# sMedX/FaceNet

Measured on AMD Instinct MI355X. Metric: images/sec (160x160 triplet train), higher is better.
Workload: dtype bf16

## Files before the change

### facenet_amd/csrc/common.h

```cpp
#pragma once
#include <hip/hip_runtime.h>
#include <stdint.h>
#include <atomic>
#include <cstdlib>

namespace fn {

enum { FN_OK = 0, FN_EINVAL = -1, FN_ELAUNCH = -2, FN_EUNSUPPORTED = -3 };
void set_error(const char* fmt, ...);
int check_launch(const char* what);

#define FN_REQUIRE(cond, ...)                  \
    do {                                       \
        if (!(cond)) {                         \
            fn::set_error(__VA_ARGS__);        \
            return fn::FN_EINVAL;              \
        }                                      \
    } while (0)

typedef __attribute__((ext_vector_type(8))) __bf16 bf16x8;
typedef __attribute__((ext_vector_type(4))) __bf16 bf16x4;
typedef __attribute__((ext_vector_type(8))) _Float16 f16x8;
typedef __attribute__((ext_vector_type(4))) _Float16 f16x4;
typedef __attribute__((ext_vector_type(4))) float f32x4;
// ... 19 lines not shown
    static __device__ __forceinline__ f32x4 mfma(vec8 a, vec8 b, f32x4 c) {
        return __builtin_amdgcn_mfma_f32_16x16x32_bf16(a, b, c, 0, 0, 0);
    }
};
template <> struct LP<_Float16> {
    typedef f16x8 vec8;
    typedef f16x4 vec4;
    static __device__ __forceinline__ float to_f32(unsigned short b) { return (float)__builtin_bit_cast(_Float16, b); }
    static __device__ __forceinline__ unsigned short from_f32(float f) {
        _Float16 h = (_Float16)f;
        return __builtin_bit_cast(unsigned short, h);
    }
    static __device__ __forceinline__ f32x4 mfma(vec8 a, vec8 b, f32x4 c) {
        return __builtin_amdgcn_mfma_f32_16x16x32_f16(a, b, c, 0, 0, 0);
    }
};

template <typename T> __device__ __forceinline__ void unpack8(const u32x4& v, float (&f)[8]) {
#pragma unroll
    for (int i = 0; i < 4; ++i) {
        f[2 * i] = LP<T>::to_f32((unsigned short)(v[i] & 0xffffu));
        f[2 * i + 1] = LP<T>::to_f32((unsigned short)(v[i] >> 16));
    }
}
template <typename T> __device__ __forceinline__ u32x4 pack8(const float (&f)[8]) {
    u32x4 v;
#pragma unroll
    for (int i = 0; i < 4; ++i)
        v[i] = (unsigned)LP<T>::from_f32(f[2 * i]) | ((unsigned)LP<T>::from_f32(f[2 * i + 1]) << 16);
    return v;
}

__device__ __forceinline__ void fast_divmod(int m, int d, float inv, int& q, int& r) {
    q = (int)((float)m * inv);
    r = m - q * d;
    const int lo = r < 0 ? 1 : 0, hi = r >= d ? 1 : 0;
    q += hi - lo;
    r += (lo - hi) * d;
}

__device__ __forceinline__ float wave_sum(float v) {
#pragma unroll
    for (int o = 32; o > 0; o >>= 1) v += __shfl_xor(v, o);
    return v;
}
__device__ __forceinline__ float wave_max(float v) {
#pragma unroll
    for (int o = 32; o > 0; o >>= 1) v = fmaxf(v, __shfl_xor(v, o));
    return v;
}

typedef int64_t acc_t;
enum { ACC_STAT = 20, ACC_GRAD = 40 };
template <int FRAC> __device__ __forceinline__ void acc_add(acc_t* p, float v) {
    atomicAdd(reinterpret_cast<unsigned long long*>(p), (unsigned long long)__double2ll_rn((double)v * (double)(1ll << FRAC)));
}
template <int FRAC> __device__ __forceinline__ float acc_get(acc_t a) { return (float)((double)a * (1.0 / (double)(1ll << FRAC))); }

__device__ __forceinline__ void bn_affine_from_sums(float s1, float s2, int count, float eps, float beta, float& scale, float& shift,
                                                    float& mean, float& var) {
#pragma clang fp contract(off)
    const float inv = 1.f / (float)count;
    mean = s1 * inv;
    const float ex2 = s2 * inv, m2 = mean * mean;
    var = fmaxf(ex2 - m2, 0.f);
    scale = rsqrtf(var + eps);
    const float ms = mean * scale;
    shift = beta - ms;
}

__device__ __forceinline__ float bn_moving_update(float moving, float batch, float momentum) {
#pragma clang fp contract(off)
    const float a = moving * momentum, w = 1.f - momentum;
    const float b = batch * w;
    return a + b;
}

__device__ __forceinline__ void bn_batch_affine(const acc_t* __restrict__ stats, int c, int sq_off, int reps, int rep_stride, int count,
                                                float eps, float beta, float& scale, float& shift, float& mean, float& var) {
    acc_t s = 0, q = 0;
    for (int rp = 0; rp < reps; ++rp) {
        s += stats[(long)rp * rep_stride + c];
        q += stats[(long)rp * rep_stride + sq_off + c];
    }
    bn_affine_from_sums(acc_get<ACC_STAT>(s), acc_get<ACC_STAT>(q), count, eps, beta, scale, shift, mean, var);
}

enum { STORE_WT = 17 };
__device__ __forceinline__ __amdgpu_buffer_rsrc_t wt_rsrc(const void* base) {
    return __builtin_amdgcn_make_buffer_rsrc(const_cast<void*>(base), 0, 0x7fffffff, 0x00020000);
}
__device__ __forceinline__ void store_wt(const __amdgpu_buffer_rsrc_t rs, long byte_offset, u32x4 v) {
    __builtin_amdgcn_raw_buffer_store_b128(v, rs, (int)byte_offset, 0, STORE_WT);
}

__device__ __forceinline__ int xcd_remap(int bid, int nwg) {
    const int q = nwg >> 3, r = nwg & 7, x = bid & 7;
    const int base = (x < r) ? x * (q + 1) : r * (q + 1) + (x - r) * q;
    return base + (bid >> 3);
}

static inline int cdiv(long a, long b) { return (int)((a + b - 1) / b); }

static inline int env_int(const char* name, int dflt) {
    const char* v = getenv(name);
    return v ? atoi(v) : dflt;
}

struct LdsOptIn {
    std::atomic<bool> done[32];
};
static inline int allow_big_lds(const void* kernel, LdsOptIn& state, const char* what) {
    int dev = 0;
    if (hipGetDevice(&dev) != hipSuccess || dev < 0 || dev >= 32) {
        set_error("%s: no current HIP device (or more than 32 devices)", what);
        return FN_ELAUNCH;
    }
    if (state.done[dev].load(std::memory_order_relaxed)) return FN_OK;
    const hipError_t e = hipFuncSetAttribute(kernel, hipFuncAttributeMaxDynamicSharedMemorySize, 160 * 1024);
    if (e != hipSuccess) {
        set_error("%s: hipFuncSetAttribute(MaxDynamicSharedMemorySize, 160 KiB) failed on device %d: %s", what, dev, hipGetErrorString(e));
        return FN_ELAUNCH;
    }
    state.done[dev].store(true, std::memory_order_relaxed);
    return FN_OK;
}

static __global__ void fill_words_kernel(unsigned* __restrict__ p, unsigned v0, unsigned v1, int n) {
    for (int i = blockIdx.x * blockDim.x + threadIdx.x; i < n; i += gridDim.x * blockDim.x) p[i] = (i & 1) ? v1 : v0;
}
static inline void fill_words(void* p, unsigned v0, unsigned v1, int n, hipStream_t st) {
    hipLaunchKernelGGL(fill_words_kernel, dim3(n > 4096 ? 16 : 1), dim3(256), 0, st, (unsigned*)p, v0, v1, n);
}

}
```

### facenet_amd/csrc/elementwise.hip

```cpp
#include "common.h"
#include "../../include/facenet_hip.h"

namespace fn {

__device__ __forceinline__ unsigned f2ord(float f) {
    unsigned u = __float_as_uint(f);
    return (u & 0x80000000u) ? ~u : (u | 0x80000000u);
}
__device__ __forceinline__ float ord2f(unsigned u) {
    return __uint_as_float((u & 0x80000000u) ? (u & 0x7fffffffu) : ~u);
}

template <typename SRC>
__global__ __launch_bounds__(256) void img_stats_kernel(const SRC* __restrict__ img, unsigned* __restrict__ work, int count) {
    const int n = blockIdx.y;
    const SRC* p = img + (long)n * count;
    float mx = -3e38f, mn = 3e38f, s = 0.f, q = 0.f;
    constexpr int PER = 16 / sizeof(SRC);
    const int head = min(count, (int)(((16 - ((uintptr_t)p & 15)) & 15) / sizeof(SRC)));
    const int nvec = (count - head) / PER;
    const SRC* pv = p + head;
    for (int i = blockIdx.x * 256 + threadIdx.x; i < nvec; i += gridDim.x * 256) {
        const u32x4 v = *reinterpret_cast<const u32x4*>(pv + (long)i * PER);
#pragma unroll
        for (int w = 0; w < 4; ++w) {
            if constexpr (sizeof(SRC) == 1) {
#pragma unroll
                for (int b = 0; b < 4; ++b) {
                    const float x = (float)((v[w] >> (8 * b)) & 0xffu);
                    mx = fmaxf(mx, x); mn = fminf(mn, x); s += x; q += x * x;
                }
            } else {
                const float x = __uint_as_float(v[w]);
                mx = fmaxf(mx, x); mn = fminf(mn, x); s += x; q += x * x;
            }
        }
    }
    if (blockIdx.x == 0) {
        for (int i = threadIdx.x; i < head; i += 256) {
            const float x = (float)p[i];
            mx = fmaxf(mx, x); mn = fminf(mn, x); s += x; q += x * x;
        }
        for (int i = head + nvec * PER + threadIdx.x; i < count; i += 256) {
            const float x = (float)p[i];
            mx = fmaxf(mx, x); mn = fminf(mn, x); s += x; q += x * x;
        }
    }
    mx = wave_max(mx); mn = -wave_max(-mn); s = wave_sum(s); q = wave_sum(q);
    if ((threadIdx.x & 63) == 0) {
        atomicMax(&work[8 * n + 0], f2ord(mx));
        atomicMax(&work[8 * n + 1], f2ord(-mn));
        acc_add<ACC_STAT>(reinterpret_cast<acc_t*>(&work[8 * n + 2]), s);
        acc_add<ACC_STAT>(reinterpret_cast<acc_t*>(&work[8 * n + 4]), q);
    }
}

template <typename T, typename SRC>
__global__ __launch_bounds__(256) void img_apply_kernel(const SRC* __restrict__ img, unsigned short* __restrict__ out,
                                                        const unsigned* __restrict__ work, int HW, int mode) {
    const int n = blockIdx.y;
    float mul, sub, den;
    if (mode == 0) {
        const float mx = ord2f(work[8 * n + 0]), mn = -ord2f(work[8 * n + 1]);
        mul = 2.f; sub = mn + mx; den = fmaxf(mx - mn, 1e-3f);
    } else {
        const float cnt = (float)HW * 3.f;
        const float mean = acc_get<ACC_STAT>(*reinterpret_cast<const acc_t*>(&work[8 * n + 2])) / cnt;
        const float var = fmaxf(acc_get<ACC_STAT>(*reinterpret_cast<const acc_t*>(&work[8 * n + 4])) / cnt - mean * mean, 0.f);
        mul = 1.f; sub = mean; den = fmaxf(sqrtf(var), rsqrtf(cnt));
    }
    const SRC* p = img + (long)n * HW * 3;
    unsigned short* o = out + (long)n * HW * 8;
    for (int px = blockIdx.x * 256 + threadIdx.x; px < HW; px += gridDim.x * 256) {
        float v[8] = {0, 0, 0, 0, 0, 0, 0, 0};
#pragma unroll
        for (int c = 0; c < 3; ++c) v[c] = (mul * (float)p[px * 3 + c] - sub) / den;
        *reinterpret_cast<u32x4*>(o + (long)px * 8) = pack8<T>(v);
    }
}

template <typename SRC>
__global__ __launch_bounds__(256) void resize_bilinear_kernel(const SRC* __restrict__ img, float* __restrict__ out, int N, int H, int W,
                                                              int OH, int OW) {
    const float sy = (float)H / (float)OH, sx = (float)W / (float)OW;
    const long total = (long)N * OH * OW;
    for (long t = (long)blockIdx.x * 256 + threadIdx.x; t < total; t += (long)gridDim.x * 256) {
        const int ox = (int)(t % OW);
        const int oy = (int)((t / OW) % OH);
        const int n = (int)(t / ((long)OW * OH));
        const float fy = ((float)oy + 0.5f) * sy - 0.5f, fx = ((float)ox + 0.5f) * sx - 0.5f;
        const float fy0 = floorf(fy), fx0 = floorf(fx);
        const int y0 = max((int)fy0, 0), y1 = min((int)ceilf(fy), H - 1);
        const int x0 = max((int)fx0, 0), x1 = min((int)ceilf(fx), W - 1);
        const float ly = fy - fy0, lx = fx - fx0;
        const SRC* p = img + (long)n * H * W * 3;
#pragma unroll
        for (int c = 0; c < 3; ++c) {
            const float v00 = (float)p[((long)y0 * W + x0) * 3 + c], v01 = (float)p[((long)y0 * W + x1) * 3 + c];
            const float v10 = (float)p[((long)y1 * W + x0) * 3 + c], v11 = (float)p[((long)y1 * W + x1) * 3 + c];
            const float top = v00 + (v01 - v00) * lx, bot = v10 + (v11 - v10) * lx;
            out[t * 3 + c] = top + (bot - top) * ly;
        }
    }
}

__global__ __launch_bounds__(256) void gather_images_kernel(const uint8_t* __restrict__ pool, const int32_t* __restrict__ idx,
                                                            uint8_t* __restrict__ out, int bytes) {
    const int i = blockIdx.y;
    const uint8_t* s = pool + (long)idx[i] * bytes;
    uint8_t* d = out + (long)i * bytes;
    const int nvec = bytes >> 4;
    for (int k = blockIdx.x * 256 + threadIdx.x; k < nvec; k += gridDim.x * 256)
        reinterpret_cast<u32x4*>(d)[k] = reinterpret_cast<const u32x4*>(s)[k];
}

template <typename T>
__global__ __launch_bounds__(256) void bn_relu_fwd_kernel(const unsigned short* __restrict__ y, int ld_y, unsigned short* __restrict__ z,
                                                          int ld_z, int M, int C, const acc_t* __restrict__ stats, int sq_off, int reps, int rep_stride,
                                                          const float* __restrict__ beta, float* __restrict__ save_scale,
                                                          float* __restrict__ save_shift, float* __restrict__ mm, float* __restrict__ mv,
                                                          float momentum, float eps, int relu, int rows_per_block) {
    __shared__ float s_scale[64], s_shift[64];
    __shared__ acc_t s_part[4][2][64];
    const int lin_ = xcd_remap(blockIdx.x + blockIdx.y * gridDim.x, gridDim.x * gridDim.y);
    const int bx_ = lin_ / gridDim.y, by_ = lin_ - bx_ * gridDim.y;
    const int c0 = by_ * 64;
    const int ncg = min(8, (C - c0) >> 3);
    const int TX = ncg <= 1 ? 1 : (ncg <= 2 ? 2 : (ncg <= 4 ? 4 : 8));
    const int TY = 256 / TX;
    const int tx = threadIdx.x % TX, ty = threadIdx.x / TX;
    const int r0 = bx_ * rows_per_block, r1 = min(M, r0 + rows_per_block);
// ... 584 lines not shown
    float s = 0.f, d = 0.f;
    for (int k = lane; k < E; k += 64) {
        const float v = x[(long)row * E + k];
        s += v * v;
        d += v * dout[(long)row * E + k];
    }
    s = wave_sum(s);
    d = wave_sum(d);
    const bool clamped = s < eps;
    const float r = rsqrtf(fmaxf(s, eps));
    for (int k = lane; k < E; k += 64) {
        const float v = x[(long)row * E + k];
        dx[(long)row * E + k] = clamped ? r * dout[(long)row * E + k] : r * (dout[(long)row * E + k] - v * r * r * d);
    }
}

template <typename T> __global__ __launch_bounds__(256) void cast_kernel(const float* __restrict__ x, unsigned short* __restrict__ y, long n) {
    for (long i = (long)blockIdx.x * 256 + threadIdx.x; i < n; i += (long)gridDim.x * 256) y[i] = LP<T>::from_f32(x[i]);
}

static inline int reduce_rows_per_block(int M, int C) {
    int chunks = 32768 / (C > 0 ? C : 1);
    if (chunks < 8) chunks = 8;
    if (chunks > 1024) chunks = 1024;
    int rpb = cdiv(M, chunks);
    if (rpb < 32) rpb = 32;
    return rpb;
}

static inline int grid_for(long work_items, int per_block = 256, int cap = 4096) {
    long g = (work_items + per_block - 1) / per_block;
    if (g < 1) g = 1;
    if (g > cap) g = cap;
    return (int)g;
}

}

using namespace fn;
#define DT_CHECK(dt) FN_REQUIRE((dt) == FN_BF16 || (dt) == FN_F16, "dtype %d unsupported", (dt))
#define LAUNCH_T(dt, KERN, grid, block, smem, st, ...)                                             \
    do {                                                                                             \
        if ((dt) == FN_BF16) hipLaunchKernelGGL(KERN<__bf16>, grid, block, smem, st, __VA_ARGS__);   \
        else hipLaunchKernelGGL(KERN<_Float16>, grid, block, smem, st, __VA_ARGS__);                 \
    } while (0)

template <typename SRC>
static int image_normalize_impl(const SRC* img, void* out, float* work, int N, int HW, int mode, int dtype, void* stream) {
    DT_CHECK(dtype);
    FN_REQUIRE(img && out && work && N > 0 && HW > 0, "image_normalize: bad arguments");
    FN_REQUIRE(mode == 0 || mode == 1, "Invalid image normalization algorithm");
    FN_REQUIRE(((uintptr_t)img % sizeof(SRC)) == 0, "image_normalize: misaligned images");
    hipStream_t st = (hipStream_t)stream;
    fill_words(work, 0u, 0u, 8 * N, st);
    hipLaunchKernelGGL(img_stats_kernel<SRC>, dim3(8, N), dim3(256), 0, st, img, (unsigned*)work, HW * 3);
    const int gx = grid_for(HW, 256, 32);
    if (dtype == FN_BF16) hipLaunchKernelGGL((img_apply_kernel<__bf16, SRC>), dim3(gx, N), dim3(256), 0, st, img, (unsigned short*)out, (const unsigned*)work, HW, mode);
    else hipLaunchKernelGGL((img_apply_kernel<_Float16, SRC>), dim3(gx, N), dim3(256), 0, st, img, (unsigned short*)out, (const unsigned*)work, HW, mode);
    return check_launch("image_normalize");
}
extern "C" int fn_image_normalize(const uint8_t* img, void* out, float* work, int N, int HW, int mode, int dtype, void* stream) {
    return image_normalize_impl<uint8_t>(img, out, work, N, HW, mode, dtype, stream);
}
extern "C" int fn_image_normalize_f32(const float* img, void* out, float* work, int N, int HW, int mode, int dtype, void* stream) {
    return image_normalize_impl<float>(img, out, work, N, HW, mode, dtype, stream);
}

extern "C" int fn_image_resize_bilinear(const void* img, int src_is_f32, float* out, int N, int H, int W, int OH, int OW, void* stream) {
    FN_REQUIRE(img && out && N > 0 && H > 0 && W > 0 && OH > 0 && OW > 0, "image_resize: bad arguments");
    const int grid = grid_for((long)N * OH * OW);
    if (src_is_f32) hipLaunchKernelGGL(resize_bilinear_kernel<float>, dim3(grid), dim3(256), 0, (hipStream_t)stream, (const float*)img, out, N, H, W, OH, OW);
    else hipLaunchKernelGGL(resize_bilinear_kernel<uint8_t>, dim3(grid), dim3(256), 0, (hipStream_t)stream, (const uint8_t*)img, out, N, H, W, OH, OW);
    return check_launch("image_resize");
}

__global__ __launch_bounds__(256) void crop_or_pad_kernel(const uint8_t* __restrict__ src, const long long* __restrict__ off,
                                                          const int* __restrict__ hw, uint8_t* __restrict__ dst, int S) {
    const int n = blockIdx.y;
    const int h = hw[2 * n], w = hw[2 * n + 1];
    const int cy = max((h - S) / 2, 0), cx = max((w - S) / 2, 0);
    const int py = max((S - h) / 2, 0), px = max((S - w) / 2, 0);
    const int ch = min(h, S), cw = min(w, S);
    const uint8_t* im = src + off[n];
    const int words = S * S * 3 / 4;
    for (int t = blockIdx.x * 256 + threadIdx.x; t < words; t += gridDim.x * 256) {
        unsigned v = 0;
#pragma unroll
        for (int b = 0; b < 4; ++b) {
            const int e = t * 4 + b;
            const int c = e % 3, pix = e / 3;
            const int x = pix % S - px, y = pix / S - py;
            if (x >= 0 && x < cw && y >= 0 && y < ch) v |= (unsigned)im[((long)(y + cy) * w + (x + cx)) * 3 + c] << (8 * b);
        }
        reinterpret_cast<unsigned*>(dst + (long)n * S * S * 3)[t] = v;
    }
}

extern "C" int fn_crop_or_pad_u8(const uint8_t* src, const long long* offsets, const int32_t* hw, uint8_t* dst, int N, int S, void* stream) {
    FN_REQUIRE(src && offsets && hw && dst && N > 0 && S > 0 && (S * S * 3) % 4 == 0, "crop_or_pad: bad arguments");
    hipLaunchKernelGGL(crop_or_pad_kernel, dim3(cdiv(S * S * 3 / 4, 256 * 4), N), dim3(256), 0, (hipStream_t)stream, src, offsets, hw, dst, S);
    return check_launch("crop_or_pad");
}

extern "C" int fn_gather_images(const uint8_t* pool, const int32_t* idx, uint8_t* out, int n_out, int bytes, void* stream) {
    FN_REQUIRE(pool && idx && out && n_out > 0 && bytes > 0, "gather_images: bad arguments");
    FN_REQUIRE(bytes % 16 == 0, "gather_images: %d bytes per image is not a multiple of 16 (images are copied as 16-byte vectors; "
// ... 195 lines not shown
```

### facenet_amd/csrc/loss.hip

```cpp
#include "pair_tiles.h"
#include "../../include/facenet_hip.h"

namespace fn {

__global__ __launch_bounds__(256) void pairwise_kernel(const float* __restrict__ xa, const float* __restrict__ xb, float* __restrict__ out,
                                                       int* __restrict__ range, int n, int m, int E, int metric) {
    const int lane = threadIdx.x & 63, wave = threadIdx.x >> 6;
    const int i = blockIdx.y;
    const int jb = (blockIdx.x * 4 + wave) * 16;
    if (jb >= m) return;
    float a[8];
#pragma unroll
    for (int t = 0; t < 8; ++t) a[t] = (lane + 64 * t < E) ? xa[(long)i * E + lane + 64 * t] : 0.f;
    float asq = 0.f;
#pragma unroll
    for (int t = 0; t < 8; ++t) asq = __fmaf_rn(a[t], a[t], asq);
    asq = wave_sum(asq);
    DotRange seen;
    for (int j = jb; j < min(m, jb + 16); ++j) {
        float d = 0.f, bsq = 0.f;
#pragma unroll
        for (int t = 0; t < 8; ++t) {
            const float b = (lane + 64 * t < E) ? xb[(long)j * E + lane + 64 * t] : 0.f;
            d = __fmaf_rn(a[t], b, d);
            bsq = __fmaf_rn(b, b, bsq);
        }
        d = wave_sum(d);
        float r;
        if (metric == 2) {
            bsq = wave_sum(bsq);
            r = fmaxf(__fmaf_rn(-2.f, d, asq + bsq), 0.f);
        } else {
            seen.add(d);
            r = pair_distance(d, metric);
        }
        if (lane == 0) out[(long)i * m + j] = r;
    }
    if (range && lane == 0 && metric != 2) seen.write(range);
}

__device__ __forceinline__ unsigned hash_mix(unsigned h, unsigned v) {
    h ^= v;
    h ^= h >> 16;
    h *= 0x7FEB352Du;
    h ^= h >> 15;
    h *= 0x846CA68Bu;
    h ^= h >> 16;
    return h;
}
__device__ __forceinline__ unsigned hash_u32(unsigned a, unsigned b, unsigned c) {
    return hash_mix(hash_mix(hash_mix(0x9E3779B9u, a), b), c);
}

__global__ __launch_bounds__(1024) void select_pairs_kernel(const int* __restrict__ labels, int n, int* __restrict__ info) {
    __shared__ int s_lab[1024];
    __shared__ int s_off[1025];
    const int tid = threadIdx.x;
    int* rec = info + 8;
    for (int i = tid; i < n; i += 1024) s_lab[i] = labels[i];
    __syncthreads();
    int cnt = 0;
    if (tid < n)
        for (int p = tid + 1; p < n; ++p) cnt += (s_lab[p] == s_lab[tid]);
    {
        __shared__ int s_wtot[16];
        const int lane = tid & 63, wv = tid >> 6;
        int v = tid < n ? cnt : 0;
#pragma unroll
        for (int d = 1; d < 64; d <<= 1) {
            const int u = __shfl_up(v, d);
            if (lane >= d) v += u;
        }
        if (lane == 63) s_wtot[wv] = v;
        __syncthreads();
        int carry = 0;
        for (int w = 0; w < wv; ++w) carry += s_wtot[w];
        if (tid < n) s_off[tid + 1] = v + carry;
        if (tid == 0) s_off[0] = 0;
    }
    __syncthreads();
    if (tid < n) {
        int q = s_off[tid];
        for (int p = tid + 1; p < n; ++p)
            if (s_lab[p] == s_lab[tid]) { rec[5 * q + 0] = tid; rec[5 * q + 1] = p; ++q; }
    }
    if (tid == 0) {
        info[0] = s_off[n];
        info[1] = 0;
    }
// ... 32 lines not shown
        if (want < cnt) {
            const int rank = __popcll(m & ((1ull << lane) - 1ull));
            const unsigned long long sel = __ballot(hit && rank == want);
            neg = j0 + (int)__ffsll((long long)sel) - 1;
            want = -1;
        } else {
            want -= cnt;
        }
    }
    if (lane == 0) {
        rec[5 * q + 2] = neg;
        rec[5 * q + 3] = (int)hash_u32(seed, (unsigned)q, 1u);
        rec[5 * q + 4] = use_cand ? 0 : 1;
        if (use_cand) atomicAdd(&info[1], 1);
    }
}

__global__ __launch_bounds__(1024) void select_rank_kernel(int T, int* __restrict__ triplets, int* __restrict__ info) {
    const int tid = threadIdx.x;
    const int* rec = info + 8;
    const int Q = info[0];
    __shared__ unsigned long long s_key[4096];
    for (int q = tid; q < min(Q, 4096); q += 1024)
        s_key[q] = ((unsigned long long)(unsigned)rec[5 * q + 4] << 32) | (unsigned)rec[5 * q + 3];
    __syncthreads();
    for (int q = tid; q < Q; q += 1024) {
        const int cls = rec[5 * q + 4];
        const unsigned key = (unsigned)rec[5 * q + 3];
        const unsigned long long mine = ((unsigned long long)(unsigned)cls << 32) | key;
        int rank = 0;
        const int QL = min(Q, 4096);
        for (int r = 0; r < QL; ++r) {
            const unsigned long long k2 = s_key[r];
            rank += (k2 < mine || (k2 == mine && r < q)) ? 1 : 0;
        }
        for (int r = QL; r < Q; ++r) {
            const int c2 = rec[5 * r + 4];
            const unsigned k2 = (unsigned)rec[5 * r + 3];
            const bool before = (c2 < cls) || (c2 == cls && (k2 < key || (k2 == key && r < q)));
            rank += before ? 1 : 0;
        }
        if (rank < T && rec[5 * q + 2] >= 0) {
            triplets[3 * rank + 0] = rec[5 * q + 0];
            triplets[3 * rank + 1] = rec[5 * q + 1];
            triplets[3 * rank + 2] = rec[5 * q + 2];
        }
    }
    if (tid == 0) {
        info[2] = (Q < T) ? 1 : 0;
        info[3] = info[3] + 1;
    }
}

__global__ __launch_bounds__(256) void triplet_loss_kernel(const float* __restrict__ emb, float* __restrict__ demb, acc_t* __restrict__ loss,
                                                           int T, int E, float alpha) {
    const int t = blockIdx.x * 4 + (threadIdx.x >> 6), lane = threadIdx.x & 63;
    if (t >= T) return;
    const float* a = emb + (long)(3 * t) * E;
    const float* p = a + E;
    const float* ng = p + E;
    float pos = 0.f, neg = 0.f;
    for (int k = lane; k < E; k += 64) {
        const float dp = a[k] - p[k], dn = a[k] - ng[k];
        pos += dp * dp;
        neg += dn * dn;
    }
    pos = wave_sum(pos);
    neg = wave_sum(neg);
    const float l = pos - neg + alpha;
    const float on = l > 0.f ? 1.f : 0.f;
    if (lane == 0) acc_add<ACC_GRAD>(loss, fmaxf(l, 0.f) / (float)T);
    if (demb) {
        const float s = 2.f * on / (float)T;
        float* da = demb + (long)(3 * t) * E;
        for (int k = lane; k < E; k += 64) {
            da[k] = s * (ng[k] - p[k]);
            da[E + k] = s * (p[k] - a[k]);
            da[2 * E + k] = s * (a[k] - ng[k]);
        }
    }
}

template <typename T>
__global__ __launch_bounds__(256) void softmax_xent_kernel(const float* __restrict__ logits, int ld, const int* __restrict__ labels,
                                                           acc_t* __restrict__ loss, unsigned short* __restrict__ dlogits, int ld_d,
                                                           acc_t* __restrict__ dbias, int N, int C, float grad_scale) {
    __shared__ float red[4];
    const int row = blockIdx.x, tid = threadIdx.x, lane = tid & 63, wave = tid >> 6;
    const float* x = logits + (long)row * ld;
    float mx = -3e38f;
    for (int c = tid; c < C; c += 256) mx = fmaxf(mx, x[c]);
    mx = wave_max(mx);
    if (lane == 0) red[wave] = mx;
    __syncthreads();
    mx = fmaxf(fmaxf(red[0], red[1]), fmaxf(red[2], red[3]));
    __syncthreads();
    float s = 0.f;
    for (int c = tid; c < C; c += 256) s += __expf(x[c] - mx);
    s = wave_sum(s);
    if (lane == 0) red[wave] = s;
    __syncthreads();
    s = red[0] + red[1] + red[2] + red[3];
    const int lab = labels[row];
    const bool lab_ok = lab >= 0 && lab < C;
    if (tid == 0) {
        if (lab_ok) acc_add<ACC_GRAD>(loss, (logf(s) + mx - x[lab]) / (float)N);
        else reinterpret_cast<volatile unsigned*>(loss)[-1] = 1u;
    }
    if (dlogits) {
        const float inv = 1.f / s;
        unsigned short* d = dlogits + (long)row * ld_d;
        for (int c = tid; c < ld_d; c += 256) {
            float g = 0.f;
            if (c < C) {
                g = (__expf(x[c] - mx) * inv - (c == lab ? 1.f : 0.f)) * grad_scale;
                if (dbias) acc_add<ACC_GRAD>(&dbias[c], g);
            }
            d[c] = LP<T>::from_f32(g);
        }
    }
}

__global__ void loss_finish_kernel(float* loss) {
    const float v = acc_get<ACC_GRAD>(*reinterpret_cast<const acc_t*>(loss + 2));
    loss[0] = reinterpret_cast<const unsigned*>(loss)[1] ? __builtin_nanf("") : v;
}


enum { REG_FLAG = 2, REG_ACC_CENTER = 4, REG_ACC_NORM = 6 };

__device__ __forceinline__ double wave_sum_d(double v) {
#pragma unroll
// ... 204 lines not shown
    for (int c = tid; c < cols; c += 256) {
        float gz = 0.f;
        if (c < C) {
            const float r = rnorm[c], cv = margin_cosine(x[c], r);
            float D = 1.f, l = cv;
            if (c == lab) l = margin_phi(cv, k, D);
            l = k.scale * l;
            float g = (__expf(l - mx) * inv - (c == lab ? 1.f : 0.f)) * grad_scale;
            g = g * k.scale;
            g = g * D;
            if (tacc) acc_add<ACC_GRAD>(&tacc[c], g * cv);
            gz = g * r;
        }
        if (d) d[c] = LP<T>::from_f32(gz);
    }
}

__global__ __launch_bounds__(256) void margin_wgrad_fix_kernel(float* __restrict__ dw, const float* __restrict__ w, const float* __restrict__ rnorm,
                                                               acc_t* __restrict__ tacc, int C, int E) {
#pragma clang fp contract(off)
    const int j = blockIdx.x * 4 + (threadIdx.x >> 6), lane = threadIdx.x & 63;
    if (j >= C) return;
    float tf = 0.f;
    if (lane == 0) {
        tf = acc_get<ACC_GRAD>(tacc[j]);
        tacc[j] = 0;
    }
    tf = __shfl(tf, 0);
    const float r = rnorm[j];
    const float kf = (r * r) * tf;
    const float* wr = w + (long)j * E;
    float* dr = dw + (long)j * E;
    for (int e = 4 * lane; e < E; e += 256) {
        const f32x4 wv = *reinterpret_cast<const f32x4*>(wr + e);
        f32x4 dv = *reinterpret_cast<const f32x4*>(dr + e);
#pragma unroll
        for (int t = 0; t < 4; ++t) {
            const float p = kf * wv[t];
            dv[t] = dv[t] - p;
        }
        *reinterpret_cast<f32x4*>(dr + e) = dv;
    }
}
}
using namespace fn;

extern "C" int fn_pairwise_sqdist(const float* xa, const float* xb, float* out, float* range, int n, int m, int E, int metric, void* stream) {
    FN_REQUIRE(xa && xb && out && n > 0 && m > 0 && E > 0 && E <= 512, "pairwise_sqdist: bad arguments (E must be <= 512)");
    FN_REQUIRE(metric >= 0 && metric <= 2, "Undefined similarity metric %d", metric);
    hipStream_t st = (hipStream_t)stream;
    if (range) {
        fill_words(range, 0x7f7fffffu, 0x80800000u, 2, st);
    }
    hipLaunchKernelGGL(pairwise_kernel, dim3(cdiv(m, 64), n), dim3(256), 0, st, xa, xb, out, (int*)range, n, m, E, metric);
    return check_launch("pairwise_sqdist");
}

extern "C" int fn_select_triplets(const float* dist, const int32_t* labels, int n, float alpha, int nrof_triplets, uint32_t seed,
                                  int semi_hard, int32_t* triplets, int32_t* info, void* stream) {
    FN_REQUIRE(dist && labels && triplets && info && n > 1 && n <= 1024 && nrof_triplets > 0, "select_triplets: bad arguments (n <= 1024)");
    hipStream_t st = (hipStream_t)stream;
    hipLaunchKernelGGL(select_pairs_kernel, dim3(1), dim3(1024), 0, st, labels, n, info);
    const int max_pairs = n * (n - 1) / 2;
    hipLaunchKernelGGL(select_negatives_kernel, dim3(cdiv(max_pairs, 4)), dim3(256), 0, st, dist, labels, n, alpha, seed, semi_hard, info);
    hipLaunchKernelGGL(select_rank_kernel, dim3(1), dim3(1024), 0, st, nrof_triplets, triplets, info);
    return check_launch("select_triplets");
}

extern "C" int fn_triplet_loss_fwd_bwd(const float* emb, float* demb, float* loss, int T, int E, float alpha, void* stream) {
    FN_REQUIRE(emb && loss && T > 0 && E > 0, "triplet_loss: bad arguments");
    hipStream_t st = (hipStream_t)stream;
    FN_REQUIRE(((uintptr_t)loss & 7) == 0, "triplet_loss: loss must be an 8-byte aligned fp32[4]");
    fill_words(loss, 0u, 0u, 4, st);
    hipLaunchKernelGGL(triplet_loss_kernel, dim3(cdiv(T, 4)), dim3(256), 0, st, emb, demb, reinterpret_cast<acc_t*>(loss + 2), T, E, alpha);
    hipLaunchKernelGGL(loss_finish_kernel, dim3(1), dim3(1), 0, st, loss);
    return check_launch("triplet_loss");
}

extern "C" int fn_softmax_xent_fwd_bwd(const float* logits, int ld, const int32_t* labels, float* loss, void* dlogits_lp, int ld_d, fn_acc_t* dbias_,
                                       int N, int C, float grad_scale, int dtype, void* stream) {
    acc_t* dbias = reinterpret_cast<acc_t*>(dbias_);
    FN_REQUIRE(((uintptr_t)loss & 7) == 0, "softmax_xent: loss must be an 8-byte aligned fp32[4]");
    FN_REQUIRE(dtype == FN_BF16 || dtype == FN_F16, "dtype %d unsupported", dtype);
    FN_REQUIRE(logits && labels && loss && N > 0 && C > 0 && ld >= C && (!dlogits_lp || ld_d >= C), "softmax_xent: bad arguments");
    hipStream_t st = (hipStream_t)stream;
    fill_words(loss, 0u, 0u, 4, st);
    acc_t* lacc = reinterpret_cast<acc_t*>(loss + 2);
    if (dtype == FN_BF16)
        hipLaunchKernelGGL(softmax_xent_kernel<__bf16>, dim3(N), dim3(256), 0, st, logits, ld, labels, lacc, (unsigned short*)dlogits_lp, ld_d, dbias, N, C, grad_scale);
    else
        hipLaunchKernelGGL(softmax_xent_kernel<_Float16>, dim3(N), dim3(256), 0, st, logits, ld, labels, lacc, (unsigned short*)dlogits_lp, ld_d, dbias, N, C, grad_scale);
    hipLaunchKernelGGL(loss_finish_kernel, dim3(1), dim3(1), 0, st, loss);
    return check_launch("softmax_xent");
}

extern "C" int fn_center_loss_fwd_bwd(const float* x, const int32_t* labels, const float* centers, float* demb, float* terms, float* xy,
                                      int ld_xy, int N, int E, int C, float center_factor, float norm_factor, float p, void* stream) {
    FN_REQUIRE(x && labels && terms && N > 0 && E > 0 && E % 4 == 0, "center_loss: bad arguments (E must be a multiple of 4)");
    FN_REQUIRE(((uintptr_t)x & 15) == 0 && (!demb || ((uintptr_t)demb & 15) == 0) && (!centers || ((uintptr_t)centers & 15) == 0),
               "center_loss: x, demb and centers must be 16-byte aligned");
    FN_REQUIRE(((uintptr_t)terms & 7) == 0, "center_loss: terms must be an 8-byte aligned fp32[8]");
    FN_REQUIRE(!centers || C > 0, "center_loss: centers need C > 0");
    FN_REQUIRE(!xy || ld_xy > E, "center_loss: ld_xy must be > E");
    FN_REQUIRE(center_factor >= 0.f && norm_factor >= 0.f && p > 0.f, "center_loss: factors must be >= 0 and p > 0");
    hipStream_t st = (hipStream_t)stream;
    hipLaunchKernelGGL(center_loss_kernel, dim3(cdiv(N, 4)), dim3(256), 0, st, x, labels, centers, demb, terms, xy, ld_xy, N, E, C,
                       center_factor, norm_factor, p);
    hipLaunchKernelGGL(center_loss_finish_kernel, dim3(1), dim3(1), 0, st, terms);
    return check_launch("center_loss");
}

extern "C" int fn_center_update(const float* rows, int ld, int M, int E, float* centers, int C, double alfa, void* stream) {
    FN_REQUIRE(rows && centers && M > 0 && M <= 4096 && E > 0 && ld > E && C > 0, "center_update: bad arguments (M <= 4096, ld > E)");
    FN_REQUIRE(alfa >= 0.0 && alfa <= 1.0, "center_update: alfa must be in [0, 1]");
    const float k = (float)(1.0 - alfa);
    hipLaunchKernelGGL(center_update_kernel, dim3(M), dim3(256), 0, (hipStream_t)stream, rows, ld, M, E, centers, C, k);
    return check_launch("center_update");
}

extern "C" int fn_margin_weight_rnorm(const float* w, int C, int E, float eps, float* rnorm, void* stream) {
    FN_REQUIRE(w && rnorm && C > 0 && E > 0 && E % 4 == 0 && eps > 0.f, "margin_weight_rnorm: bad arguments (E must be a multiple of 4, eps > 0)");
    FN_REQUIRE(((uintptr_t)w & 15) == 0, "margin_weight_rnorm: w must be 16-byte aligned");
    hipLaunchKernelGGL(margin_rnorm_kernel, dim3(cdiv(C, 4)), dim3(256), 0, (hipStream_t)stream, w, C, E, eps, rnorm);
    return check_launch("margin_weight_rnorm");
}
// ... 30 lines not shown
```

Before: 14160.

## Collapse glue kernels into single launches for normalize, pairs, triplet loss

Several small glue ops now run as single kernels under a default-on env switch. Image normalization fuses the fill, stats and normalize passes into one kernel that accumulates stats in LDS per block. Triplet loss fuses the fill, loss and finish into one workgroup when T is small. Pair selection uses a ballot-based kernel, and pairwise distance computes four columns per wave. The aim is to cut launch count and global atomics; the cost is that every normalize block recomputes the full per-image statistics redundantly.

```diff
diff --git a/facenet_amd/csrc/common.h b/facenet_amd/csrc/common.h
--- a/facenet_amd/csrc/common.h
+++ b/facenet_amd/csrc/common.h
@@ -95,8 +95,11 @@
 
 typedef int64_t acc_t;
 enum { ACC_STAT = 20, ACC_GRAD = 40 };
+template <int FRAC> __device__ __forceinline__ unsigned long long acc_fixed(float v) {
+    return (unsigned long long)__double2ll_rn((double)v * (double)(1ll << FRAC));
+}
 template <int FRAC> __device__ __forceinline__ void acc_add(acc_t* p, float v) {
-    atomicAdd(reinterpret_cast<unsigned long long*>(p), (unsigned long long)__double2ll_rn((double)v * (double)(1ll << FRAC)));
+    atomicAdd(reinterpret_cast<unsigned long long*>(p), acc_fixed<FRAC>(v));
 }
 template <int FRAC> __device__ __forceinline__ float acc_get(acc_t a) { return (float)((double)a * (1.0 / (double)(1ll << FRAC))); }
 
@@ -150,6 +153,11 @@
     return v ? atoi(v) : dflt;
 }
 
+static inline bool glue_single_launch() {
+    static const int on = env_int("FN_GLUE_SINGLE_LAUNCH", 1);
+    return on != 0;
+}
+
 struct LdsOptIn {
     std::atomic<bool> done[32];
 };
diff --git a/facenet_amd/csrc/elementwise.hip b/facenet_amd/csrc/elementwise.hip
--- a/facenet_amd/csrc/elementwise.hip
+++ b/facenet_amd/csrc/elementwise.hip
@@ -11,16 +11,14 @@
     return __uint_as_float((u & 0x80000000u) ? (u & 0x7fffffffu) : ~u);
 }
 
+enum { IMG_STAT_SLOTS = 8 * 256 };
 template <typename SRC>
-__global__ __launch_bounds__(256) void img_stats_kernel(const SRC* __restrict__ img, unsigned* __restrict__ work, int count) {
-    const int n = blockIdx.y;
-    const SRC* p = img + (long)n * count;
-    float mx = -3e38f, mn = 3e38f, s = 0.f, q = 0.f;
+__device__ __forceinline__ void img_stats_slot(const SRC* __restrict__ p, int count, int slot, float& mx, float& mn, float& s, float& q) {
     constexpr int PER = 16 / sizeof(SRC);
     const int head = min(count, (int)(((16 - ((uintptr_t)p & 15)) & 15) / sizeof(SRC)));
     const int nvec = (count - head) / PER;
     const SRC* pv = p + head;
-    for (int i = blockIdx.x * 256 + threadIdx.x; i < nvec; i += gridDim.x * 256) {
+    for (int i = slot; i < nvec; i += IMG_STAT_SLOTS) {
         const u32x4 v = *reinterpret_cast<const u32x4*>(pv + (long)i * PER);
 #pragma unroll
         for (int w = 0; w < 4; ++w) {
@@ -36,23 +34,53 @@
             }
         }
     }
-    if (blockIdx.x == 0) {
-        for (int i = threadIdx.x; i < head; i += 256) {
+    if (slot < 256) {
+        for (int i = slot; i < head; i += 256) {
             const float x = (float)p[i];
             mx = fmaxf(mx, x); mn = fminf(mn, x); s += x; q += x * x;
         }
-        for (int i = head + nvec * PER + threadIdx.x; i < count; i += 256) {
+        for (int i = head + nvec * PER + slot; i < count; i += 256) {
             const float x = (float)p[i];
             mx = fmaxf(mx, x); mn = fminf(mn, x); s += x; q += x * x;
         }
     }
+}
+
+__device__ __forceinline__ void img_stats_publish(unsigned* w8, float mx, float mn, float s, float q) {
     mx = wave_max(mx); mn = -wave_max(-mn); s = wave_sum(s); q = wave_sum(q);
     if ((threadIdx.x & 63) == 0) {
-        atomicMax(&work[8 * n + 0], f2ord(mx));
-        atomicMax(&work[8 * n + 1], f2ord(-mn));
-        acc_add<ACC_STAT>(reinterpret_cast<acc_t*>(&work[8 * n + 2]), s);
-        acc_add<ACC_STAT>(reinterpret_cast<acc_t*>(&work[8 * n + 4]), q);
-    }
+        atomicMax(&w8[0], f2ord(mx));
+        atomicMax(&w8[1], f2ord(-mn));
+        acc_add<ACC_STAT>(reinterpret_cast<acc_t*>(&w8[2]), s);
+        acc_add<ACC_STAT>(reinterpret_cast<acc_t*>(&w8[4]), q);
+    }
+}
+
+template <typename SRC>
+__global__ __launch_bounds__(256) void img_stats_kernel(const SRC* __restrict__ img, unsigned* __restrict__ work, int count) {
+    const int n = blockIdx.y;
+    float mx = -3e38f, mn = 3e38f, s = 0.f, q = 0.f;
+    img_stats_slot<SRC>(img + (long)n * count, count, blockIdx.x * 256 + threadIdx.x, mx, mn, s, q);
+    img_stats_publish(&work[8 * n], mx, mn, s, q);
+}
+
+__device__ __forceinline__ void img_norm_coeffs(const unsigned* w8, int HW, int mode, float& mul, float& sub, float& den) {
+    if (mode == 0) {
+        const float mx = ord2f(w8[0]), mn = -ord2f(w8[1]);
+        mul = 2.f; sub = mn + mx; den = fmaxf(mx - mn, 1e-3f);
+    } else {
+        const float cnt = (float)HW * 3.f;
+        const float mean = acc_get<ACC_STAT>(*reinterpret_cast<const acc_t*>(&w8[2])) / cnt;
+        const float var = fmaxf(acc_get<ACC_STAT>(*reinterpret_cast<const acc_t*>(&w8[4])) / cnt - mean * mean, 0.f);
+        mul = 1.f; sub = mean; den = fmaxf(sqrtf(var), rsqrtf(cnt));
+    }
+}
+template <typename T, typename SRC>
+__device__ __forceinline__ void img_norm_pixel(const SRC* __restrict__ p, unsigned short* __restrict__ o, int px, float mul, float sub, float den) {
+    float v[8] = {0, 0, 0, 0, 0, 0, 0, 0};
+#pragma unroll
+    for (int c = 0; c < 3; ++c) v[c] = (mul * (float)p[px * 3 + c] - sub) / den;
+    *reinterpret_cast<u32x4*>(o + (long)px * 8) = pack8<T>(v);
 }
 
 template <typename T, typename SRC>
@@ -60,23 +88,32 @@
                                                         const unsigned* __restrict__ work, int HW, int mode) {
     const int n = blockIdx.y;
     float mul, sub, den;
-    if (mode == 0) {
-        const float mx = ord2f(work[8 * n + 0]), mn = -ord2f(work[8 * n + 1]);
-        mul = 2.f; sub = mn + mx; den = fmaxf(mx - mn, 1e-3f);
-    } else {
-        const float cnt = (float)HW * 3.f;
-        const float mean = acc_get<ACC_STAT>(*reinterpret_cast<const acc_t*>(&work[8 * n + 2])) / cnt;
-        const float var = fmaxf(acc_get<ACC_STAT>(*reinterpret_cast<const acc_t*>(&work[8 * n + 4])) / cnt - mean * mean, 0.f);
-        mul = 1.f; sub = mean; den = fmaxf(sqrtf(var), rsqrtf(cnt));
-    }
+    img_norm_coeffs(&work[8 * n], HW, mode, mul, sub, den);
     const SRC* p = img + (long)n * HW * 3;
     unsigned short* o = out + (long)n * HW * 8;
-    for (int px = blockIdx.x * 256 + threadIdx.x; px < HW; px += gridDim.x * 256) {
-        float v[8] = {0, 0, 0, 0, 0, 0, 0, 0};
-#pragma unroll
-        for (int c = 0; c < 3; ++c) v[c] = (mul * (float)p[px * 3 + c] - sub) / den;
-        *reinterpret_cast<u32x4*>(o + (long)px * 8) = pack8<T>(v);
-    }
+    for (int px = blockIdx.x * 256 + threadIdx.x; px < HW; px += gridDim.x * 256) img_norm_pixel<T, SRC>(p, o, px, mul, sub, den);
+}
+
+template <typename T, typename SRC>
+__global__ __launch_bounds__(1024) void img_normalize_kernel(const SRC* __restrict__ img, unsigned short* __restrict__ out,
+                                                            unsigned* __restrict__ work, int HW, int mode) {
+    __shared__ alignas(8) unsigned s_w8[8];
+    const int n = blockIdx.y, tid = threadIdx.x, count = HW * 3;
+    const SRC* p = img + (long)n * count;
+    if (tid < 8) s_w8[tid] = 0u;
+    __syncthreads();
+#pragma unroll
+    for (int k = 0; k < 2; ++k) {
+        float mx = -3e38f, mn = 3e38f, s = 0.f, q = 0.f;
+        img_stats_slot<SRC>(p, count, k * 1024 + tid, mx, mn, s, q);
+        img_stats_publish(s_w8, mx, mn, s, q);
+    }
+    __syncthreads();
+    if (blockIdx.x == 0 && tid < 8) work[8 * n + tid] = s_w8[tid];
+    float mul, sub, den;
+    img_norm_coeffs(s_w8, HW, mode, mul, sub, den);
+    unsigned short* o = out + (long)n * HW * 8;
+    for (int px = blockIdx.x * 1024 + tid; px < HW; px += gridDim.x * 1024) img_norm_pixel<T, SRC>(p, o, px, mul, sub, den);
 }
 
 template <typename SRC>
@@ -767,6 +804,12 @@
     FN_REQUIRE(mode == 0 || mode == 1, "Invalid image normalization algorithm");
     FN_REQUIRE(((uintptr_t)img % sizeof(SRC)) == 0, "image_normalize: misaligned images");
     hipStream_t st = (hipStream_t)stream;
+    if (glue_single_launch()) {
+        const dim3 grid(max(1, min(8, 256 / N)), N);
+        if (dtype == FN_BF16) hipLaunchKernelGGL((img_normalize_kernel<__bf16, SRC>), grid, dim3(1024), 0, st, img, (unsigned short*)out, (unsigned*)work, HW, mode);
+        else hipLaunchKernelGGL((img_normalize_kernel<_Float16, SRC>), grid, dim3(1024), 0, st, img, (unsigned short*)out, (unsigned*)work, HW, mode);
+        return check_launch("image_normalize");
+    }
     fill_words(work, 0u, 0u, 8 * N, st);
     hipLaunchKernelGGL(img_stats_kernel<SRC>, dim3(8, N), dim3(256), 0, st, img, (unsigned*)work, HW * 3);
     const int gx = grid_for(HW, 256, 32);
diff --git a/facenet_amd/csrc/loss.hip b/facenet_amd/csrc/loss.hip
--- a/facenet_amd/csrc/loss.hip
+++ b/facenet_amd/csrc/loss.hip
@@ -35,6 +35,50 @@
             r = pair_distance(d, metric);
         }
         if (lane == 0) out[(long)i * m + j] = r;
+    }
+    if (range && lane == 0 && metric != 2) seen.write(range);
+}
+
+enum { PW_COLS = 4 };
+__global__ __launch_bounds__(256) void pairwise_cols_kernel(const float* __restrict__ xa, const float* __restrict__ xb, float* __restrict__ out,
+                                                            int* __restrict__ range, int n, int m, int E, int metric) {
+    const int lane = threadIdx.x & 63, wave = threadIdx.x >> 6;
+    const int i = blockIdx.y;
+    const int jb = (blockIdx.x * 4 + wave) * PW_COLS;
+    if (jb >= m) return;
+    float a[8], b[PW_COLS][8];
+#pragma unroll
+    for (int t = 0; t < 8; ++t) a[t] = (lane + 64 * t < E) ? xa[(long)i * E + lane + 64 * t] : 0.f;
+#pragma unroll
+    for (int c = 0; c < PW_COLS; ++c) {
+        const int j = min(jb + c, m - 1);
+#pragma unroll
+        for (int t = 0; t < 8; ++t) b[c][t] = (lane + 64 * t < E) ? xb[(long)j * E + lane + 64 * t] : 0.f;
+    }
+    float asq = 0.f;
+#pragma unroll
+    for (int t = 0; t < 8; ++t) asq = __fmaf_rn(a[t], a[t], asq);
+    asq = wave_sum(asq);
+    DotRange seen;
+#pragma unroll
+    for (int c = 0; c < PW_COLS; ++c) {
+        if (jb + c >= m) break;
+        float d = 0.f, bsq = 0.f;
+#pragma unroll
+        for (int t = 0; t < 8; ++t) {
+            d = __fmaf_rn(a[t], b[c][t], d);
+            bsq = __fmaf_rn(b[c][t], b[c][t], bsq);
+        }
+        d = wave_sum(d);
+        float r;
+        if (metric == 2) {
+            bsq = wave_sum(bsq);
+            r = fmaxf(__fmaf_rn(-2.f, d, asq + bsq), 0.f);
+        } else {
+            seen.add(d);
+            r = pair_distance(d, metric);
+        }
+        if (lane == 0) out[(long)i * m + jb + c] = r;
     }
     if (range && lane == 0 && metric != 2) seen.write(range);
 }
@@ -173,10 +217,67 @@
     }
 }
 
-__global__ __launch_bounds__(256) void triplet_loss_kernel(const float* __restrict__ emb, float* __restrict__ demb, acc_t* __restrict__ loss,
-                                                           int T, int E, float alpha) {
-    const int t = blockIdx.x * 4 + (threadIdx.x >> 6), lane = threadIdx.x & 63;
-    if (t >= T) return;
+enum { SEL_PAIRS_MAX_N = 256, SEL_PAIRS_CHUNKS = SEL_PAIRS_MAX_N / 64 };
+__global__ __launch_bounds__(1024) void select_pairs_ballot_kernel(const int* __restrict__ labels, int n, int* __restrict__ info) {
+    __shared__ int s_lab[SEL_PAIRS_MAX_N];
+    __shared__ int s_off[SEL_PAIRS_MAX_N + 1];
+    __shared__ int s_wtot[16];
+    const int tid = threadIdx.x, lane = tid & 63, wv = tid >> 6;
+    int* rec = info + 8;
+    if (tid < n) s_lab[tid] = labels[tid];
+    int labk[SEL_PAIRS_CHUNKS];
+#pragma unroll
+    for (int k = 0; k < SEL_PAIRS_CHUNKS; ++k) labk[k] = labels[min(64 * k + lane, n - 1)];
+    __syncthreads();
+    for (int a = wv; a < n; a += 16) {
+        const int la = s_lab[a];
+        int cnt = 0;
+#pragma unroll
+        for (int k = 0; k < SEL_PAIRS_CHUNKS; ++k) {
+            const int j = 64 * k + lane;
+            cnt += __popcll(__ballot((j < n) && (labk[k] == la) && (j > a)));
+        }
+        if (lane == 0) s_off[a + 1] = cnt;
+    }
+    __syncthreads();
+    {
+        int v = tid < n ? s_off[tid + 1] : 0;
+#pragma unroll
+        for (int d = 1; d < 64; d <<= 1) {
+            const int u = __shfl_up(v, d);
+            if (lane >= d) v += u;
+        }
+        if (lane == 63) s_wtot[wv] = v;
+        __syncthreads();
+        int carry = 0;
+        for (int w = 0; w < wv; ++w) carry += s_wtot[w];
+        if (tid < n) s_off[tid + 1] = v + carry;
+        if (tid == 0) s_off[0] = 0;
+    }
+    __syncthreads();
+    for (int a = wv; a < n; a += 16) {
+        const int la = s_lab[a];
+        int q = s_off[a];
+#pragma unroll
+        for (int k = 0; k < SEL_PAIRS_CHUNKS; ++k) {
+            const int j = 64 * k + lane;
+            const bool pos = (j < n) && (labk[k] == la) && (j > a);
+            const unsigned long long m = __ballot(pos);
+            if (pos) {
+                const int idx = q + __popcll(m & ((1ull << lane) - 1ull));
+                rec[5 * idx + 0] = a;
+                rec[5 * idx + 1] = j;
+            }
+            q += __popcll(m);
+        }
+    }
+    if (tid == 0) {
+        info[0] = s_off[n];
+        info[1] = 0;
+    }
+}
+
+__device__ __forceinline__ float triplet_one(const float* __restrict__ emb, float* __restrict__ demb, int t, int lane, int T, int E, float alpha) {
     const float* a = emb + (long)(3 * t) * E;
     const float* p = a + E;
     const float* ng = p + E;
@@ -190,7 +291,6 @@
     neg = wave_sum(neg);
     const float l = pos - neg + alpha;
     const float on = l > 0.f ? 1.f : 0.f;
-    if (lane == 0) acc_add<ACC_GRAD>(loss, fmaxf(l, 0.f) / (float)T);
     if (demb) {
         const float s = 2.f * on / (float)T;
         float* da = demb + (long)(3 * t) * E;
@@ -199,6 +299,35 @@
             da[E + k] = s * (p[k] - a[k]);
             da[2 * E + k] = s * (a[k] - ng[k]);
         }
+    }
+    return fmaxf(l, 0.f) / (float)T;
+}
+
+__global__ __launch_bounds__(256) void triplet_loss_kernel(const float* __restrict__ emb, float* __restrict__ demb, acc_t* __restrict__ loss,
+                                                           int T, int E, float alpha) {
+    const int t = blockIdx.x * 4 + (threadIdx.x >> 6), lane = threadIdx.x & 63;
+    if (t >= T) return;
+    const float term = triplet_one(emb, demb, t, lane, T, E, alpha);
+    if (lane == 0) acc_add<ACC_GRAD>(loss, term);
+}
+
+enum { TRIPLET_ONE_WG_MAX = 64 };
+__global__ __launch_bounds__(1024) void triplet_loss_one_wg_kernel(const float* __restrict__ emb, float* __restrict__ demb, float* __restrict__ loss,
+                                                                  int T, int E, float alpha) {
+    __shared__ unsigned long long s_acc;
+    const int lane = threadIdx.x & 63, wv = threadIdx.x >> 6;
+    if (threadIdx.x == 0) s_acc = 0ull;
+    __syncthreads();
+    for (int t = wv; t < T; t += 16) {
+        const float term = triplet_one(emb, demb, t, lane, T, E, alpha);
+        if (lane == 0) atomicAdd(&s_acc, acc_fixed<ACC_GRAD>(term));
+    }
+    __syncthreads();
+    if (threadIdx.x == 0) {
+        const acc_t acc = (acc_t)s_acc;
+        loss[0] = acc_get<ACC_GRAD>(acc);
+        reinterpret_cast<unsigned*>(loss)[1] = 0u;
+        *reinterpret_cast<acc_t*>(loss + 2) = acc;
     }
 }
 
@@ -509,7 +638,8 @@
     if (range) {
         fill_words(range, 0x7f7fffffu, 0x80800000u, 2, st);
     }
-    hipLaunchKernelGGL(pairwise_kernel, dim3(cdiv(m, 64), n), dim3(256), 0, st, xa, xb, out, (int*)range, n, m, E, metric);
+    if (glue_single_launch()) hipLaunchKernelGGL(pairwise_cols_kernel, dim3(cdiv(m, 4 * PW_COLS), n), dim3(256), 0, st, xa, xb, out, (int*)range, n, m, E, metric);
+    else hipLaunchKernelGGL(pairwise_kernel, dim3(cdiv(m, 64), n), dim3(256), 0, st, xa, xb, out, (int*)range, n, m, E, metric);
     return check_launch("pairwise_sqdist");
 }
 
@@ -517,7 +647,8 @@
                                   int semi_hard, int32_t* triplets, int32_t* info, void* stream) {
     FN_REQUIRE(dist && labels && triplets && info && n > 1 && n <= 1024 && nrof_triplets > 0, "select_triplets: bad arguments (n <= 1024)");
     hipStream_t st = (hipStream_t)stream;
-    hipLaunchKernelGGL(select_pairs_kernel, dim3(1), dim3(1024), 0, st, labels, n, info);
+    if (glue_single_launch() && n <= SEL_PAIRS_MAX_N) hipLaunchKernelGGL(select_pairs_ballot_kernel, dim3(1), dim3(1024), 0, st, labels, n, info);
+    else hipLaunchKernelGGL(select_pairs_kernel, dim3(1), dim3(1024), 0, st, labels, n, info);
     const int max_pairs = n * (n - 1) / 2;
     hipLaunchKernelGGL(select_negatives_kernel, dim3(cdiv(max_pairs, 4)), dim3(256), 0, st, dist, labels, n, alpha, seed, semi_hard, info);
     hipLaunchKernelGGL(select_rank_kernel, dim3(1), dim3(1024), 0, st, nrof_triplets, triplets, info);
@@ -528,6 +659,10 @@
     FN_REQUIRE(emb && loss && T > 0 && E > 0, "triplet_loss: bad arguments");
     hipStream_t st = (hipStream_t)stream;
     FN_REQUIRE(((uintptr_t)loss & 7) == 0, "triplet_loss: loss must be an 8-byte aligned fp32[4]");
+    if (glue_single_launch() && T <= TRIPLET_ONE_WG_MAX) {
+        hipLaunchKernelGGL(triplet_loss_one_wg_kernel, dim3(1), dim3(1024), 0, st, emb, demb, loss, T, E, alpha);
+        return check_launch("triplet_loss");
+    }
     fill_words(loss, 0u, 0u, 4, st);
     hipLaunchKernelGGL(triplet_loss_kernel, dim3(cdiv(T, 4)), dim3(256), 0, st, emb, demb, reinterpret_cast<acc_t*>(loss + 2), T, E, alpha);
     hipLaunchKernelGGL(loss_finish_kernel, dim3(1), dim3(1), 0, st, loss);
```

Result: no change. 14240, median of 6 (+0.5%).
